# xeTaiz/vit-tf

Measured on AMD Instinct MI355X. Metric: slices/sec (ViT-S/8, 512^3 vol: feature volume + 16-query similarity), higher is better.
Workload: dtype fp16; 1 GPU; 512^3 CT-like synthetic volume (seed 0), ViT-S/8, fos 64: 1536 slices of 512x512 (N=4097) per step + 16-query similarity -> the metric's configuration (BASELINE configs[2]); engine_batch=512, weights=seeded synthetic vits8 (seed 0), parallelism=single GPU

## Files before the change

### vit-tf_amd/csrc/tail_fx.hip

```cpp
#include "vittf_common.h"

#include <type_traits>
#include <utility>

namespace {

constexpr int D = 384, HID = 4 * D, UNITS = HID / 32;
constexpr int SB = 24576, HB = SB / 2;
constexpr int PSTEPS = D / 32;
constexpr int LAG = 4;
constexpr int MSTEPS = 2 * UNITS + LAG;
constexpr int NSEQ = PSTEPS + MSTEPS;
constexpr int NSLOT = 4, AHEAD = NSLOT - 1;
constexpr int PIECES = SB / 1024 / 4;
constexpr int WAIT0 = (AHEAD - 2) * PIECES;
constexpr int NF = 4;
constexpr int PB_OFF = NSLOT * SB;
constexpr int PBH = 4608, PB = 2 * PBH;
constexpr int STG_ROW = 144;
constexpr int AF_SLOT = 1056, AF_H = 528;
constexpr int CONST_OFF = PB_OFF + 4 * PB;
constexpr int C_B1 = 0, C_B2 = HID, C_G1 = HID + D, C_E1 = HID + 2 * D,
              C_BP = HID + 3 * D, C_G2 = HID + 4 * D, C_E2 = HID + 5 * D,
              C_N = HID + 6 * D;
// ... 177 lines not shown
#define FX_ROLE_ENV                                                                                                       \
  const unsigned short* const abuf = uni_ptr(c.abuf);                                                                     \
  float* const x = uni_ptr(c.x);                                                                                          \
  unsigned short* const hout = uni_ptr(c.hout);                                                                           \
  unsigned* const tile_ctr = uni_ptr(c.tile_ctr);                                                                         \
  const int64_t rows = (int64_t)(((uint64_t)uni((unsigned)((uint64_t)c.rows >> 32)) << 32) | uni((unsigned)c.rows));     \
  const float ln_eps = __uint_as_float(uni(__float_as_uint(c.ln_eps)));                                                   \
  const int ntiles = (int)uni((unsigned)c.ntiles);                                                                        \
  int tile = (int)uni((unsigned)c.tile);                                                                                  \
  const unsigned lds0 = uni(c.lds0);                                                                                      \
  const int tid = threadIdx.x;                                                                                            \
  const int lane = tid & 63, wave = __builtin_amdgcn_readfirstlane(tid >> 6);                                             \
  const int rb = wave & 3;                                                                                                \
  const int h = lane >> 5, l31 = lane & 31;                                                                               \
  unsigned cl = lds0 + CONST_OFF + 16 * h;                                                                                \
  asm volatile("" : "+v"(cl));                                                                                            \
  auto cst4 = [&](int i) { return *(lds_f4_ptr)(cl + 4 * i); };             \
  const unsigned nxt = lds0 + NEXT_OFF;                                                                                   \
  Ring st;                                                                                                                \
  st.rsrc = lds_dma_rsrc(uni_ptr(c.wpk), (unsigned)(NSEQ * SB));                                                          \
  st.src0 = rb * (PIECES * 1024);                                                                                         \
  st.dma_dst = lds0;                                                                                                      \
  st.g = 0;                                                                                                               \
  st.slot = 0;                                                                                                            \
  const int aoff0 = tile_off(l31, h);                                                                                     \
  const unsigned pbuf = lds0 + PB_OFF + rb * PB;                           \
   \
  auto tile_rsrc = [&](const void* p, int64_t tile, int row_bytes) {                                                      \
    const int64_t first = tile * 128, left = rows - first;                                                                \
    const int nrows = tile < 0 || left <= 0 || !p ? 0 : left < 128 ? (int)left : 128;                                     \
    return __builtin_amdgcn_make_buffer_rsrc(const_cast<char*>(reinterpret_cast<const char*>(p)) + (nrows ? first : 0) * row_bytes, 0, \
                                             nrows * row_bytes, 0x00020000);                                              \
  };                                                                                                                      \
  (void)abuf; (void)x; (void)hout; (void)tile_ctr; (void)ln_eps; (void)ntiles; (void)l31; (void)aoff0; (void)nxt; (void)cst4; (void)tile_rsrc

template <int DT>
__device__ __attribute__((noinline)) void run_f(Ctx c) {
  FX_ROLE_ENV;
  asm volatile("s_setprio 3");
  unsigned pbl = pbuf + lane * 16;
  asm volatile("" : "+v"(pbl));
  u32x4_t fb[48];
  const int q8 = lane >> 3, c8 = lane & 7;
  __amdgpu_buffer_rsrc_t ra, rx;
  const int ao = (rb * 32 + q8) * (D * 2) + c8 * 16, xo = (rb * 32 + q8) * (D * 4) + c8 * 16;
  auto load_a = [&](int cg) {
#pragma unroll
    for (int i = 0; i < 4; ++i) fb[4 * cg + i] = __builtin_amdgcn_raw_buffer_load_b128(ra, ao + cg * 128, i * 8 * (D * 2), 0);
  };
  auto load_chunk = [&](int c) {
    const int r0 = c < 6 ? 24 + 4 * c : 4 * (c - 6);
#pragma unroll
    for (int i = 0; i < 4; ++i) fb[r0 + i] = __builtin_amdgcn_raw_buffer_load_b128(rx, xo + c * 128, i * 8 * (D * 4), 0);
  };
  const unsigned af_wr = pbuf + (c8 >> 1) * AF_SLOT + (c8 & 1) * AF_H + q8 * 16;
  auto put_a = [&](int cg) {
#pragma unroll
    for (int i = 0; i < 4; ++i) *(lds_wu4_ptr)(af_wr + af_off(4 * cg) + i * 128) = fb[4 * cg + i];
  };
  const unsigned ch_wr = pbuf + q8 * STG_ROW + c8 * 16;
  auto put_chunk = [&](int c) {
    const int r0 = c < 6 ? 24 + 4 * c : 4 * (c - 6);
#pragma unroll
    for (int i = 0; i < 4; ++i) *(lds_wu4_ptr)(ch_wr + (c & 1) * PBH + i * 8 * STG_ROW) = fb[r0 + i];
  };
  auto fetch_rows = [&](int t) {
    ra = tile_rsrc(abuf, t, D * 2);
    rx = tile_rsrc(x, t, D * 4);
#pragma unroll
    for (int cg = 0; cg < 6; ++cg) load_a(cg);
#pragma unroll
    for (int c = 0; c < 6; ++c) load_chunk(c);
    put_a(0);
  };
  fetch_rows(tile);
  asm volatile("s_waitcnt vmcnt(0)" ::: "memory");
  __syncthreads();
  while (true) {
    unsigned next_v = 0;
    if (tid == 256) next_v = atomicAdd(tile_ctr, 1u);
    unsigned base[4];
    s16x8_t hf[D / 16];
    s16x8_t wf[NF];
    f32x16_t bias_c;
    auto load_bias = [&](int at) {
#pragma unroll
      for (int q = 0; q < 4; ++q) {
        const f32x4_t bv = cst4(at + 8 * q);
        bias_c[4 * q + 0] = bv[0]; bias_c[4 * q + 1] = bv[1]; bias_c[4 * q + 2] = bv[2]; bias_c[4 * q + 3] = bv[3];
      }
    };
#pragma unroll
    for (int p = 0; p < PSTEPS; ++p) {
      sync_wait<true>();
      if (p % 2 == 0 && p / 2 + 1 < 6) put_a(p / 2 + 1);
      if (p == 0) load_chunk(6);
      if (p % 2 == 1 && p / 2 < 5) load_chunk(7 + p / 2);
      if (p == PSTEPS - 1) put_chunk(0);
      ring_advance(st);
    }
#pragma unroll
    for (int r = 0; r < 12; ++r) {
      sync_wait<true>();
      if (r + 1 < 12) put_chunk(r + 1);
    }
#pragma unroll
    for (int r = 0; r < 12; ++r) {
      sync_wait<true>();
// ... 19 lines not shown
      __builtin_amdgcn_sched_barrier(0);
    }
    ring_advance(st);
    f_step<DT, 1, false, false, false>(st, base, wf, hf, ga, bias_c, gb, pk1);
    for (int u = 1; u < UNITS - 1; u += 2) {
      load_bias(C_B1 + 32 * u);
      f_step<DT, 0, true, false, true>(st, base, wf, hf, gb, bias_c, ga, pk0);
      f_step<DT, 1, true, false, false>(st, base, wf, hf, gb, bias_c, ga, pk1);
      put_gf(0);
      load_bias(C_B1 + 32 * (u + 1));
      f_step<DT, 0, true, false, true>(st, base, wf, hf, ga, bias_c, gb, pk0);
      f_step<DT, 1, true, false, false>(st, base, wf, hf, ga, bias_c, gb, pk1);
      put_gf(1);
    }
    load_bias(C_B1 + 32 * (UNITS - 1));
    f_step<DT, 0, true, false, true>(st, base, wf, hf, gb, bias_c, ga, pk0);
    f_step<DT, 1, true, true, false>(st, base, wf, hf, gb, bias_c, ga, pk1);
    put_gf(0);
    sync_wait<true>();
    ring_advance(st);
#pragma unroll
    for (int r = 0; r < 16; r += 2) {
      const float v0 = gelu_poly(gb[r]), v1 = gelu_poly(gb[r + 1]);
      const unsigned w = pack2_h16<DT>(v0, v1);
      if (r < 8) pk0[r >> 1] = w; else pk1[(r - 8) >> 1] = w;
    }
    put_gf(1);
    sync_wait<true>(); ring_advance(st);
    sync_wait(); ring_advance(st);
    sync_wait(); ring_advance(st);
    if (tid == 256) *(lds_u32_ptr)nxt = next_v;
    asm volatile("s_waitcnt vmcnt(0) lgkmcnt(0)\n\ts_barrier" ::: "memory");
    const int next = __builtin_amdgcn_readfirstlane((int)*(lds_u32_ptr)nxt);
    if (next >= ntiles) break;
    tile = next;
    fetch_rows(tile);
  }
}

template <int DT>
__device__ __attribute__((noinline)) void run_x(Ctx c) {
  FX_ROLE_ENV;
  unsigned base[4];
  asm volatile("s_waitcnt vmcnt(0)" ::: "memory");
  __syncthreads();
  s16x8_t wf[NF];
  f32x16_t xacc[D / 32];
  while (true) {
    int ln = lane;
    asm volatile("" : "+v"(ln));
    {
#pragma unroll
      for (int ot = 0; ot < D / 32; ++ot)
#pragma unroll
        for (int q = 0; q < 4; ++q) {
          const f32x4_t bv = cst4(C_BP + 32 * ot + 8 * q);
          xacc[ot][4 * q + 0] = bv[0]; xacc[ot][4 * q + 1] = bv[1]; xacc[ot][4 * q + 2] = bv[2]; xacc[ot][4 * q + 3] = bv[3];
        }
#pragma unroll
      for (int i = 0; i < 4; ++i) base[i] = lds0 + st.slot * SB + (aoff0 ^ (32 * i));
      const unsigned af_rd = pbuf + (ln >> 5) * AF_H + (ln & 31) * 16;
      s16x8_t aa[2], ab[2];
      x_wait<-1, true>();
#pragma unroll
      for (int f = 0; f < NF; ++f) wf[f] = ld_frag(base, f);
      aa[0] = *(lds_frag_ptr)(af_rd + af_off(0));
      aa[1] = *(lds_frag_ptr)(af_rd + af_off(1));
      p_step<DT, -1, true, false>(st, base, wf, xacc, aa, ab, af_rd + af_off(2), af_rd + af_off(3));
      p_step<DT, -1, false, false>(st, base, wf, xacc, ab, aa, af_rd + af_off(4), af_rd + af_off(5));
// ... 64 lines not shown
          }
          *(lds_wu4_ptr)(hw_ + (ot & 1) * PBH + k2 * 1024) = pk;
        }
        sync_wait<true>();
      }
    }
    s16x8_t gf[2];
    x_idle_step<WAIT0>(st); x_idle_step<WAIT0>(st); x_idle_step<WAIT0>(st);
    x_wait<WAIT0>();
    {
      const int g_next = ring_next(st), slot_free = ring_free(st);
#pragma unroll
      for (int i = 0; i < PIECES; ++i) ring_piece(st, i, g_next, slot_free);
      ring_advance(st);
#pragma unroll
      for (int i = 0; i < 4; ++i) base[i] = lds0 + st.slot * SB + HB + (aoff0 ^ (32 * i));
#pragma unroll
      for (int f = 0; f < NF; ++f) wf[f] = ld_frag(base, f);
    }
    const unsigned gfa = pbuf + ln * 16;
    for (int u = 0; u < UNITS - 2; u += 2) {
      x_step<DT, 0, false>(st, base, wf, xacc, gf, gfa);
      x_step<DT, 1, false>(st, base, wf, xacc, gf, gfa);
      x_step<DT, 0, false>(st, base, wf, xacc, gf, gfa + PBH);
      x_step<DT, 1, false>(st, base, wf, xacc, gf, gfa + PBH);
    }
    x_step<DT, 0, false>(st, base, wf, xacc, gf, gfa);
    x_step<DT, 1, false>(st, base, wf, xacc, gf, gfa);
    x_step<DT, 0, false>(st, base, wf, xacc, gf, gfa + PBH);
    x_step<DT, 1, true>(st, base, wf, xacc, gf, gfa + PBH);
    asm volatile("s_waitcnt vmcnt(0) lgkmcnt(0)\n\ts_barrier" ::: "memory");
    const int next = __builtin_amdgcn_readfirstlane((int)*(lds_u32_ptr)nxt);
    {
      const auto rxo = tile_rsrc(x, tile, D * 4);
      const auto rho = tile_rsrc(hout, tile, D * 2);
      int le = lane;
      asm volatile("" : "+v"(le));
      const unsigned stg_wr_e = pbuf + (le & 31) * STG_ROW + 16 * (le >> 5);
      const unsigned stg_wh = pbuf + (le & 31) * STG_ROW + 8 * (le >> 5);
      const unsigned stg_rd_e = pbuf + (le >> 3) * STG_ROW + (le & 7) * 16;
      const int xo_e = (rb * 32 + (le >> 3)) * (D * 4) + (le & 7) * 16;
      const int ho = (rb * 32 + (le >> 3)) * (D * 2) + (le & 7) * 16;
      float s = 0.f;
      {
        f32x4_t bvq[2][4];
#pragma unroll
        for (int g = 0; g < 4; ++g) bvq[0][g] = cst4(C_B2 + 8 * g);
#pragma unroll
        for (int ot = 0; ot < D / 32; ++ot) {
#pragma unroll
          for (int g = 0; g < 4; ++g) {
            const f32x4_t bv = bvq[ot & 1][g];
            f32x4_t v;
            v[0] = xacc[ot][4 * g + 0] + bv[0]; v[1] = xacc[ot][4 * g + 1] + bv[1];
            v[2] = xacc[ot][4 * g + 2] + bv[2]; v[3] = xacc[ot][4 * g + 3] + bv[3];
#pragma unroll
            for (int e = 0; e < 4; ++e) xacc[ot][4 * g + e] = v[e];
            *(lds_w4_ptr)(stg_wr_e + 32 * g) = v;
            s += (v[0] + v[1]) + (v[2] + v[3]);
          }
          __builtin_amdgcn_sched_barrier(0);
          f32x4_t rbk[4];
#pragma unroll
          for (int i = 0; i < 4; ++i) rbk[i] = *(lds_f4_ptr)(stg_rd_e + i * 8 * STG_ROW);
          if (ot + 1 < D / 32) {
#pragma unroll
            for (int g = 0; g < 4; ++g) bvq[(ot + 1) & 1][g] = cst4(C_B2 + 32 * (ot + 1) + 8 * g);
          }
          __builtin_amdgcn_sched_barrier(0);
#pragma unroll
          for (int i = 0; i < 4; ++i)
            __builtin_amdgcn_raw_buffer_store_b128(__builtin_bit_cast(u32x4_t, rbk[i]), rxo, xo_e + ot * 128, i * 8 * (D * 4), 0);
          __builtin_amdgcn_sched_barrier(0);
        }
      }
      if (hout) {
        {
          const auto sw = __builtin_amdgcn_permlane32_swap(__float_as_uint(s), __float_as_uint(s), false, false);
          s = __uint_as_float(sw[0]) + __uint_as_float(sw[1]);
        }
        const float mean = s / (float)D;
        float q = 0.f;
#pragma unroll
        for (int ot = 0; ot < D / 32; ++ot) {
#pragma unroll
          for (int r = 0; r < 16; ++r) { const float dv = xacc[ot][r] - mean; q += dv * dv; }
          __builtin_amdgcn_sched_barrier(0);
        }
        {
          const auto sw = __builtin_amdgcn_permlane32_swap(__float_as_uint(q), __float_as_uint(q), false, false);
          q = __uint_as_float(sw[0]) + __uint_as_float(sw[1]);
        }
        const float rstd = 1.0f / sqrtf(q / (float)D + ln_eps);
        float mean_p = mean;
        asm volatile("" : "+v"(mean_p));
        f32x4_t gq1[2][4], bq1[2][4];
#pragma unroll
        for (int g = 0; g < 4; ++g) { gq1[0][g] = cst4(C_G1 + 8 * g); bq1[0][g] = cst4(C_E1 + 8 * g); }
#pragma unroll
        for (int ot = 0; ot < D / 32; ++ot) {
          const int op = ot >> 1, o2 = ot & 1;
#pragma unroll
          for (int g = 0; g < 4; ++g) {
            const f32x4_t gg = gq1[ot & 1][g], bb = bq1[ot & 1][g];
            u32x2_t pk;
            pk[0] = pack2_h16<DT>((xacc[ot][4 * g + 0] - mean_p) * rstd * gg[0] + bb[0], (xacc[ot][4 * g + 1] - mean_p) * rstd * gg[1] + bb[1]);
            pk[1] = pack2_h16<DT>((xacc[ot][4 * g + 2] - mean_p) * rstd * gg[2] + bb[2], (xacc[ot][4 * g + 3] - mean_p) * rstd * gg[3] + bb[3]);
            *(lds_w2_ptr)(stg_wh + 64 * o2 + 16 * g) = pk;
          }
          __builtin_amdgcn_sched_barrier(0);
          [[maybe_unused]] f32x4_t rbk[4];
          if (o2) {
#pragma unroll
            for (int i = 0; i < 4; ++i) rbk[i] = *(lds_f4_ptr)(stg_rd_e + i * 8 * STG_ROW);
          }
          if (ot + 1 < D / 32) {
#pragma unroll
            for (int g = 0; g < 4; ++g) { gq1[(ot + 1) & 1][g] = cst4(C_G1 + 32 * (ot + 1) + 8 * g); bq1[(ot + 1) & 1][g] = cst4(C_E1 + 32 * (ot + 1) + 8 * g); }
          }
          __builtin_amdgcn_sched_barrier(0);
          if (o2) {
#pragma unroll
            for (int i = 0; i < 4; ++i)
              __builtin_amdgcn_raw_buffer_store_b128(__builtin_bit_cast(u32x4_t, rbk[i]), rho, ho + op * 128, i * 8 * (D * 2), 0);
            __builtin_amdgcn_sched_barrier(0);
          }
        }
      }
    }
    if (next >= ntiles) break;
    tile = next;
  }
}

template <int DT>
__global__ __launch_bounds__(512, 1) void tail_fx_kernel(const unsigned short* __restrict__ abuf, const unsigned short* __restrict__ wpk,
                                                         const float* __restrict__ bp, const float* __restrict__ g2, const float* __restrict__ e2,
                                                         const float* __restrict__ b1, const float* __restrict__ b2,
                                                         float* __restrict__ x, int64_t rows, const float* __restrict__ ln_g,
                                                         const float* __restrict__ ln_b, float ln_eps,
                                                         unsigned short* __restrict__ hout, int ntiles,
                                                         unsigned* __restrict__ tile_ctr) {
  __shared__ __attribute__((aligned(16))) char smem[LDS_BYTES];
  const int tid = threadIdx.x;
  const int lane = tid & 63, wave = __builtin_amdgcn_readfirstlane(tid >> 6);
  float* const cst = reinterpret_cast<float*>(smem + CONST_OFF);
  for (int i = tid; i < C_N; i += 512) {
    float v;
    if (i < C_B2) v = b1[i];
    else if (i < C_G1) v = b2[i - C_B2];
    else if (i < C_E1) v = ln_g ? ln_g[i - C_G1] : 1.f;
    else if (i < C_BP) v = ln_b ? ln_b[i - C_E1] : 0.f;
    else if (i < C_G2) v = bp[i - C_BP];
    else if (i < C_E2) v = g2[i - C_G2];
    else v = e2[i - C_E2];
    cst[i] = v;
  }
  const unsigned lds0 = (unsigned)(size_t)LDS_PTR(smem);
  const unsigned nxt = lds0 + NEXT_OFF;
  if (tid == 0) *(lds_u32_ptr)nxt = atomicAdd(tile_ctr, 1u);
  __syncthreads();
  const int tile = __builtin_amdgcn_readfirstlane((int)*(lds_u32_ptr)nxt);
  if (tile >= ntiles) return;
  if (wave < 4) {
// ... 46 lines not shown
```

### include/vittf.h

```cpp
#ifndef VITTF_H
#define VITTF_H

#include <stddef.h>
#include <stdint.h>

#ifdef __cplusplus
extern "C" {
#endif

#define VITTF_ABI_VERSION 6

typedef enum vittf_status {
  VITTF_OK = 0,
  VITTF_ERR_INVALID_ARG = -1,
  VITTF_ERR_WORKSPACE = -2,
  VITTF_ERR_LAUNCH = -3,
  VITTF_ERR_NO_DEVICE = -4
} vittf_status;

typedef enum vittf_dtype { VITTF_BF16 = 0, VITTF_FP16 = 1 } vittf_dtype;

typedef enum vittf_axis { VITTF_AXIS_X = 0, VITTF_AXIS_Y = 1, VITTF_AXIS_Z = 2 } vittf_axis;

typedef enum vittf_sample_mode { VITTF_SAMPLE_NEAREST = 0, VITTF_SAMPLE_TRILINEAR = 1 } vittf_sample_mode;
// ... 114 lines not shown
                          float* tokens_out, void* stream);

int vittf_layernorm(const float* x, const float* g, const float* b, void* y, int64_t rows, int32_t d,
                    float eps, int32_t dtype, void* stream);

int vittf_token_features(const float* x, const float* norm_g, const float* norm_b, uint16_t* t_out, int32_t batch,
                         int32_t tokens, int32_t prefix, int32_t d, float eps, void* stream);

typedef enum vittf_epilogue {
  VITTF_EPI_BIAS = 0,
  VITTF_EPI_BIAS_GELU = 1,
  VITTF_EPI_BIAS_RESIDUAL = 2,
  VITTF_EPI_KFEAT = 3,
  VITTF_EPI_BIAS_QKV = 4
} vittf_epilogue;

int vittf_gemm(const void* a, const void* w, const float* bias, void* out, int64_t rows, int32_t n, int32_t k,
               int32_t epilogue, int32_t tokens, int32_t dtype, void* stream);

int vittf_gemm_kfeat_parts(const void* a, const void* w, const float* bias, int64_t rows, int32_t d, int32_t k,
                           int32_t tokens, int32_t part_mask, void* q_out, void* k_out, void* v_out, int32_t dtype,
                           void* stream);

int vittf_gemm_kfeat_parts_reg(const void* a, const void* w, const float* bias, int64_t rows, int32_t d, int32_t k,
                               int32_t tokens, int32_t n_reg, int32_t part_mask, void* q_out, void* k_out, void* v_out,
                               int32_t dtype, void* stream);

int vittf_gemm_residual_ln(const void* a, const void* w, const float* bias, float* x, int64_t rows, int32_t n, int32_t k,
                           int32_t dtype, const float* ln_g, const float* ln_b, float ln_eps, void* h, void* stream);

size_t vittf_gemm_as_workspace_bytes(void);
int vittf_gemm_as(const void* a, const void* w_packed, const float* bias, void* out, int64_t rows, int32_t n, int32_t k,
                  int32_t epilogue, int32_t dtype, void* tile_counter, void* stream);

size_t vittf_block_tail_workspace_bytes(void);
int vittf_block_tail(const void* attn_out, const void* w_packed, const float* proj_b, const float* ln2_g, const float* ln2_b,
                     const float* b1, const float* b2, float* x, int64_t rows, int32_t d, int32_t dtype, const float* ln_g,
                     const float* ln_b, float ln_eps, void* h_out, void* tile_counter, void* stream);

int vittf_rope_qk(void* qkv, int64_t rows, int32_t tokens, int32_t prefix, int32_t heads, const vittf_rope_table* table,
                  int32_t dtype, void* stream);

int vittf_attention(const void* qkv, void* out, int32_t batch, int32_t tokens, int32_t heads, int32_t dtype,
                    int32_t q_prescaled, void* stream);

int64_t vittf_attention_rescale_count(int32_t reset);

size_t vittf_attention_fp8_workspace_bytes(int32_t batch, int32_t tokens, int32_t heads);
int vittf_attention_fp8(const void* qkv, void* out, int32_t batch, int32_t tokens, int32_t heads, int32_t dtype, void* ws,
                        size_t ws_bytes, void* stream);

int vittf_gemm_qkv_fp8(const void* a, const void* w, const float* bias, void* qkv_out, int64_t rows, int32_t n, int32_t k,
                       int32_t tokens, int32_t heads, int32_t dtype, void* ws, size_t ws_bytes, void* stream);
int vittf_attention_fp8_rows(const void* qkv, void* out, int32_t batch, int32_t tokens, int32_t heads, int32_t dtype, void* ws,
                             size_t ws_bytes, void* stream);


int vittf_pool_slices(const uint16_t* k_slices, int32_t k_slice0, int32_t k_nslices, int32_t total_slices,
                      int32_t n_out, int32_t win0, int32_t nwin, int32_t f0, int32_t f1, int32_t d,
                      uint16_t* dst, int64_t dst_stride_d, int64_t dst_stride_win, int64_t dst_stride_row,
                      int64_t dst_stride_col, void* stream);

int vittf_pool_slices3d(const uint16_t* k_slices, int32_t k_slice0, int32_t k_nslices, int32_t total_slices,
                        int32_t n_out, int32_t win0, int32_t nwin, int32_t f0, int32_t f1, int32_t d,
                        uint16_t* dst, int64_t dst_stride_d, int64_t dst_stride_win, int64_t dst_stride_row,
                        int64_t dst_stride_col, int32_t o0, int32_t o1, int32_t slice_dim, void* stream);
// ... 94 lines not shown
```

### vit-tf_amd/_lib.py

```python
import ctypes as C
import os

_HERE = os.path.dirname(os.path.abspath(__file__))
LIB_PATH = os.path.join(_HERE, 'libvittf.so')

BF16, FP16 = 0, 1
DTYPES = {'bf16': BF16, 'bfloat16': BF16, 'fp16': FP16, 'float16': FP16, 'half': FP16}
SAMPLE_MODES = {'nearest': 0, 'bilinear': 1, 'trilinear': 1}
EPI_BIAS, EPI_BIAS_GELU, EPI_BIAS_RESIDUAL, EPI_KFEAT, EPI_BIAS_QKV = 0, 1, 2, 3, 4


class VitConfig(C.Structure):
    _fields_ = [('embed_dim', C.c_int32), ('depth', C.c_int32), ('heads', C.c_int32), ('patch', C.c_int32),
                ('dtype', C.c_int32), ('ln_eps', C.c_float), ('attention_fp8', C.c_int32), ('flags', C.c_int32)]


CFG_SEPARATE_LN, CFG_UNSCALED_Q, CFG_FP8_HEAD_SCALES = 1, 2, 4


class VitWeights(C.Structure):
    _fields_ = [(n, C.c_void_p) for n in (
        'pe_w_t', 'pe_b', 'qkv_w', 'qkv_b', 'proj_w', 'proj_b', 'fc1_w', 'fc1_b', 'fc2_w', 'fc2_b', 'tail_packed', 'qkv_packed',
        'ln1_g', 'ln1_b', 'ln2_g', 'ln2_b')]

# ... 28 lines not shown
SIGNATURES = {
    'vittf_abi_version': (C.c_int, []),
    'vittf_status_string': (C.c_char_p, [C.c_int]),
    'vittf_device_count': (C.c_int, []),
    'vittf_minmax_workspace_bytes': (_sz, []),
    'vittf_volume_minmax': (C.c_int, [_vp, _i64, _vp, _vp, _sz, _vp]),
    'vittf_vit_workspace_bytes': (_sz, [_P(VitConfig), _i32, _i32]),
    'vittf_vit_k_features': (C.c_int, [_P(VitConfig), _P(VitWeights), _P(PosEmbed), _P(SliceView), _i32, _i32, _i32,
                                       _vp, _vp, _sz, _vp]),
    'vittf_vit_qkv_features': (C.c_int, [_P(VitConfig), _P(VitWeights), _P(PosEmbed), _P(SliceView), _i32, _i32, _i32,
                                         _vp, _vp, _vp, _vp, _sz, _vp]),
    'vittf_vit_qkv_features_reg': (C.c_int, [_P(VitConfig), _P(VitWeights), _P(PosEmbed), _P(SliceView), _i32, _i32, _i32,
                                             _vp, _i32, _vp, _vp, _vp, _vp, _sz, _vp]),
    'vittf_vit_qkv_features_rope': (C.c_int, [_P(VitConfig), _P(VitWeights), _P(PosEmbed), _P(SliceView), _i32, _i32, _i32,
                                              _vp, _i32, _P(RopeTable), _vp, _vp, _vp, _vp, _sz, _vp]),
    'vittf_vit_features': (C.c_int, [_P(VitConfig), _P(VitWeights), _P(PosEmbed), _P(SliceView), _i32, _i32, _i32, _vp, _i32,
                                     _P(RopeTable), _vp, _vp, _vp, _vp, _vp, _vp, _vp, _sz, _vp]),
    'vittf_profiler_enable': (C.c_int, [_i32]),
    'vittf_profiler_collect': (C.c_int, [_P(C.c_double), _P(_i64)]),
    'vittf_profiler_kernel_name': (C.c_char_p, [_i32]),
    'vittf_patch_embed': (C.c_int, [_P(VitConfig), _P(VitWeights), _P(PosEmbed), _P(SliceView), _i32, _i32, _vp, _vp]),
    'vittf_patch_embed_reg': (C.c_int, [_P(VitConfig), _P(VitWeights), _P(PosEmbed), _P(SliceView), _i32, _i32, _vp, _i32, _vp,
                                        _vp]),
    'vittf_token_features': (C.c_int, [_vp, _vp, _vp, _vp, _i32, _i32, _i32, _i32, C.c_float, _vp]),
    'vittf_layernorm': (C.c_int, [_vp, _vp, _vp, _vp, _i64, _i32, C.c_float, _i32, _vp]),
    'vittf_gemm': (C.c_int, [_vp, _vp, _vp, _vp, _i64, _i32, _i32, _i32, _i32, _i32, _vp]),
    'vittf_gemm_kfeat_parts': (C.c_int, [_vp, _vp, _vp, _i64, _i32, _i32, _i32, _i32, _vp, _vp, _vp, _i32, _vp]),
    'vittf_gemm_kfeat_parts_reg': (C.c_int, [_vp, _vp, _vp, _i64, _i32, _i32, _i32, _i32, _i32, _vp, _vp, _vp, _i32, _vp]),
    'vittf_gemm_residual_ln': (C.c_int, [_vp, _vp, _vp, _vp, _i64, _i32, _i32, _i32, _vp, _vp, C.c_float, _vp, _vp]),
    'vittf_block_tail_workspace_bytes': (_sz, []),
    'vittf_block_tail': (C.c_int, [_vp, _vp, _vp, _vp, _vp, _vp, _vp, _vp, _i64, _i32, _i32, _vp, _vp, C.c_float, _vp, _vp, _vp]),
    'vittf_gemm_as_workspace_bytes': (_sz, []),
    'vittf_gemm_as': (C.c_int, [_vp, _vp, _vp, _vp, _i64, _i32, _i32, _i32, _i32, _vp, _vp]),
    'vittf_rope_qk': (C.c_int, [_vp, _i64, _i32, _i32, _i32, _P(RopeTable), _i32, _vp]),
    'vittf_attention': (C.c_int, [_vp, _vp, _i32, _i32, _i32, _i32, _i32, _vp]),
    'vittf_attention_rescale_count': (_i64, [_i32]),
    'vittf_attention_fp8_workspace_bytes': (_sz, [_i32, _i32, _i32]),
    'vittf_attention_fp8': (C.c_int, [_vp, _vp, _i32, _i32, _i32, _i32, _vp, _sz, _vp]),
    'vittf_gemm_qkv_fp8': (C.c_int, [_vp, _vp, _vp, _vp, _i64, _i32, _i32, _i32, _i32, _i32, _vp, _sz, _vp]),
    'vittf_attention_fp8_rows': (C.c_int, [_vp, _vp, _i32, _i32, _i32, _i32, _vp, _sz, _vp]),
    'vittf_pool_slices': (C.c_int, [_vp, _i32, _i32, _i32, _i32, _i32, _i32, _i32, _i32, _i32, _vp, _i64, _i64, _i64,
                                    _i64, _vp]),
    'vittf_pool_slices3d': (C.c_int, [_vp, _i32, _i32, _i32, _i32, _i32, _i32, _i32, _i32, _i32, _vp, _i64, _i64, _i64,
                                      _i64, _i32, _i32, _i32, _vp]),
    'vittf_assemble_sum': (C.c_int, [_vp, _vp, _vp, _i32, _P(_i32), _i32, _i32, _i32, _i32, _vp, _vp]),
    'vittf_sample_features': (C.c_int, [_vp, _i32, _i32, _i32, _i32, _i32, _vp, _i32, _i32, _vp, _vp, _vp]),
    'vittf_voxel_norm': (C.c_int, [_vp, _i32, _i64, _vp, _vp]),
    'vittf_similarity_workspace_bytes': (_sz, [_i32, _i64, _i32]),
    'vittf_similarity': (C.c_int, [_vp, _i32, _i32, _i32, _i32, _vp, _P(_i32), _i32, _i32, _vp, _i32, _i32, _i32, _vp, _vp,
                                   _sz, _vp]),
    'vittf_similarity_query_workspace_bytes': (_sz, [_i32, _i64, _i32, _i32]),
    'vittf_similarity_query': (C.c_int, [_vp, _i32, _i32, _i32, _i32, _P(C.c_float), _P(_i32), _i32, _i32, _vp, _i32, _i32, _i32,
                                         _vp, _vp, _sz, _vp]),
    'vittf_similarity_maps_f32': (C.c_int, [_vp, _i32, _i32, _i32, _i32, _i32, _vp, _P(_i32), _i32, _i32, C.c_float, _vp, _vp,
                                            _vp, _sz, _vp]),
    'vittf_feature_gram_workspace_bytes': (_sz, [_i32, _i64]),
    'vittf_feature_gram': (C.c_int, [_vp, _i32, _i64, _vp, _vp, _vp, _sz, _vp]),
    'vittf_feature_project': (C.c_int, [_vp, _i32, _i64, _vp, _vp, _i32, _vp, _vp]),
    'vittf_kmeans_assign': (C.c_int, [_vp, _i32, _i64, _vp, _vp, _i32, _vp, _vp, _vp]),
    'vittf_kmeans_sums_workspace_bytes': (_sz, [_i32, _i64, _i32]),
    'vittf_kmeans_sums': (C.c_int, [_vp, _i32, _i64, _vp, _i32, _vp, _vp, _vp, _sz, _vp]),
    'vittf_topk_voxels': (C.c_int, [_vp, _i32, _i64, _i32, _vp, _vp]),
    'vittf_mean_pairwise_distance': (C.c_int, [_vp, _i32, _i32, _i32, _vp, _vp]),
    'vittf_erode_mask': (C.c_int, [_vp, _i32, _i32, _i32, _i32, _i32, _vp, _vp]),
    'vittf_surface_shell_workspace_bytes': (_sz, [_i32, _i32, _i32]),
    'vittf_surface_shell': (C.c_int, [_vp, _i32, _i32, _i32, _i32, _i32, _vp, _vp, _sz, _vp]),
# ... 84 lines not shown
```

### vit-tf_amd/csrc/gemm_as.hip

```cpp
#include "vittf_common.h"

#include <stdlib.h>
#include <type_traits>

namespace {

constexpr int K = 384;
constexpr int SB = 24576;
constexpr int NSLOT = 4, AHEAD = NSLOT - 1;
constexpr int PIECES = SB / 1024 / 4;
constexpr int NF = 4;
constexpr int STG_ROW = 144, STG = 32 * STG_ROW;
constexpr int STG_OFF = NSLOT * SB;
constexpr int BIAS_OFF = STG_OFF + 12 * STG;
constexpr int MAXN = 1536;
constexpr int NEXT_OFF = BIAS_OFF + MAXN * 4;
constexpr int LDS_BYTES = NEXT_OFF + 16;
static_assert(LDS_BYTES <= 160 * 1024, "LDS");

typedef __attribute__((ext_vector_type(4))) unsigned u32x4_t;
typedef __attribute__((ext_vector_type(2))) unsigned u32x2_t;
typedef __attribute__((address_space(3))) const s16x8_t* lds_frag_ptr;
typedef __attribute__((address_space(3))) const f32x4_t* lds_f4_ptr;
typedef __attribute__((address_space(3))) u32x2_t* lds_w2_ptr;
typedef __attribute__((address_space(3))) volatile unsigned* lds_u32_ptr;

__device__ __forceinline__ void lds_dma16_keep(i32x4_t rsrc, unsigned lds_addr, int voff, int soff) {
  asm volatile("s_mov_b32 m0, %0\n\ts_nop 0\n\tbuffer_load_dwordx4 %1, %2, %3 offen lds"
               :: "s"(lds_addr), "v"(voff), "s"(rsrc), "s"(soff) : "memory");
}

template <int DT>
__global__ __launch_bounds__(512, 1) void gemm_as_kernel(const unsigned short* __restrict__ abuf, const unsigned short* __restrict__ wpk,
                                                         const float* __restrict__ bias, unsigned short* __restrict__ out, int64_t rows,
                                                         int n, int qcols, int ntiles, unsigned* __restrict__ tile_ctr) {
  __shared__ __attribute__((aligned(16))) char smem[LDS_BYTES];
  const int tid = threadIdx.x;
  const int lane = tid & 63, wave = __builtin_amdgcn_readfirstlane(tid >> 6);
  const int h = lane >> 5, l31 = lane & 31, q8 = lane >> 3, c8 = lane & 7;
  const unsigned lds0 = (unsigned)(size_t)LDS_PTR(smem);
  float* const cst = reinterpret_cast<float*>(smem + BIAS_OFF);
  for (int i = tid; i < n; i += 512) cst[i] = bias[i];
  const unsigned nxt = lds0 + NEXT_OFF;
  if (tid == 0) *(lds_u32_ptr)nxt = atomicAdd(tile_ctr, 1u);
  __syncthreads();
  int tile = __builtin_amdgcn_readfirstlane((int)*(lds_u32_ptr)nxt);
  if (tile >= ntiles) return;
  const int units = n >> 5;
  const i32x4_t rsrc = lds_dma_rsrc(wpk, (unsigned)(units * SB));
  const bool storer = wave >= 4;
  const int src0 = (wave & 3) * (PIECES * 1024);
  if (!storer) {
#pragma unroll
    for (int u = 0; u < AHEAD; ++u)
#pragma unroll
      for (int i = 0; i < PIECES; ++i)
        lds_dma16(rsrc, lds0 + u * SB + src0 + i * 1024, lane * 16, u * SB + src0 + i * 1024);
  }
  int g = 0, slot = 0;
  const int aoff0 = tile_off(l31, h);
  unsigned base[4];
#pragma unroll
  for (int i = 0; i < 4; ++i) base[i] = lds0 + (aoff0 ^ (32 * i));
  const unsigned stg = lds0 + STG_OFF + (storer ? 8 + (wave - 4) : 2 * wave) * STG;
  const unsigned stg_w = stg + l31 * STG_ROW + 8 * h;
  const unsigned stg_r = stg + q8 * STG_ROW + c8 * 16;
  const unsigned stg_rp = lds0 + STG_OFF + 2 * (wave & 3) * STG + q8 * STG_ROW + c8 * 16;
  unsigned cl = lds0 + BIAS_OFF + 16 * h;
  asm volatile("" : "+v"(cl));
  constexpr float QS = 0.125f * 1.44269504088896340736f;
  asm volatile("s_waitcnt vmcnt(0)" ::: "memory");
  __syncthreads();
  s16x8_t wf[NF];
#pragma unroll
  for (int f = 0; f < NF; ++f) wf[f] = *(lds_frag_ptr)(base[f & 3] + (f >> 2) * 4096);
  const int row_bytes_out = n * 2;

  while (true) {
    unsigned next_v = 0;
    if (tid == 256) next_v = atomicAdd(tile_ctr, 1u);
    const int64_t first = (int64_t)tile * 256, left = rows - first;
    const int nrows = left < 256 ? (int)left : 256;
    const auto ra = __builtin_amdgcn_make_buffer_rsrc(const_cast<unsigned short*>(abuf) + first * K, 0, nrows * (K * 2), 0x00020000);
    const auto ro = __builtin_amdgcn_make_buffer_rsrc(out + first * n, 0, nrows * row_bytes_out, 0x00020000);
    s16x8_t hq[K / 16];
#pragma unroll
    for (int s = 0; s < K / 16; ++s)
      hq[s] = __builtin_bit_cast(s16x8_t, __builtin_amdgcn_raw_buffer_load_b128(ra, (wave * 32 + l31) * (K * 2) + 16 * h, 32 * s, 0));
    const int oo = (wave * 32 + q8) * row_bytes_out + c8 * 16;
    f32x16_t qa = {}, qb = {};
    f32x4_t ba[4], bb[4];
    auto load_bias = [&](int u, f32x4_t (&b)[4]) {
#pragma unroll
      for (int gq = 0; gq < 4; ++gq) b[gq] = *(lds_f4_ptr)(cl + 4 * (32 * u + 8 * gq));
    };
    auto stage = [&](const f32x16_t& q, const f32x4_t (&bq)[4], int u, int gq) {
      const f32x4_t b = bq[gq];
      const float qsc = 32 * u < qcols ? QS : 1.f;
      u32x2_t pk;
      pk[0] = pack2_h16<DT>((q[4 * gq + 0] + b[0]) * qsc, (q[4 * gq + 1] + b[1]) * qsc);
      pk[1] = pack2_h16<DT>((q[4 * gq + 2] + b[2]) * qsc, (q[4 * gq + 3] + b[3]) * qsc);
      *(lds_w2_ptr)(stg_w + (storer ? 0 : ((u >> 1) & 1) * STG) + 64 * (u & 1) + 16 * gq) = pk;
    };
    auto store_pair = [&](int m, bool partner) {
      if (!storer) return;
      const unsigned rd = partner ? stg_rp + (m & 1) * STG : stg_r;
      f32x4_t rbk[4];
#pragma unroll
      for (int i = 0; i < 4; ++i) rbk[i] = *(lds_f4_ptr)(rd + i * 8 * STG_ROW);
#pragma unroll
      for (int i = 0; i < 4; ++i)
        __builtin_amdgcn_raw_buffer_store_b128(__builtin_bit_cast(u32x4_t, rbk[i]), ro, oo + (partner ? -128 * row_bytes_out : 0) + m * 128,
                                               i * 8 * row_bytes_out, 0);
    };
    auto unit = [&](auto WAITc, f32x16_t& acc, f32x4_t (&bcur)[4], const f32x16_t& prevq, const f32x4_t (&bprev)[4], int u, bool stage_prev) {
      constexpr int WAITN = decltype(WAITc)::value;
      load_bias(u, bcur);
      if (storer) asm volatile("s_waitcnt lgkmcnt(0)\n\ts_barrier" ::: "memory");
      else asm volatile("s_waitcnt vmcnt(%0) lgkmcnt(0)\n\ts_barrier" ::"i"(WAITN) : "memory");
      if (u >= 3 && (u & 1)) store_pair((u - 3) >> 1, true);
      const int g_next = g + AHEAD < units ? g + AHEAD : g + AHEAD - units;
      const int slot_free = slot == 0 ? NSLOT - 1 : slot - 1;
#pragma unroll
      for (int j = 0; j < 24; ++j) {
        acc = mfma32<DT>(wf[j % NF], hq[j], j == 0 ? f32x16_t{} : acc);
        if (j == 24 - NF) {
          const int d_ = slot == NSLOT - 1 ? -(NSLOT - 1) * SB : SB;
#pragma unroll
          for (int i = 0; i < 4; ++i) { base[i] += d_; asm volatile("" : "+v"(base[i])); }
        }
        wf[j % NF] = *(lds_frag_ptr)(base[((j + NF) % 24) & 3] + (((j + NF) % 24) >> 2) * 4096);
        if (!storer && j % 4 == 3) lds_dma16_keep(rsrc, lds0 + slot_free * SB + src0 + (j >> 2) * 1024, lane * 16, g_next * SB + src0 + (j >> 2) * 1024);
        if (stage_prev && j % 6 == 2) stage(prevq, bprev, u - 1, j / 6);
        __builtin_amdgcn_sched_barrier(0);
      }
      g = g + 1 == units ? 0 : g + 1;
      slot = slot + 1 == NSLOT ? 0 : slot + 1;
    };
    using W6 = std::integral_constant<int, PIECES>;
    using WT = std::integral_constant<int, PIECES + K / 16>;
    unit(WT{}, qa, ba, qb, bb, 0, false);
    unit(W6{}, qb, bb, qa, ba, 1, true);
    for (int u = 2; u < units; u += 2) {
      unit(W6{}, qa, ba, qb, bb, u, true);
      store_pair((u - 2) >> 1, false);
      unit(W6{}, qb, bb, qa, ba, u + 1, true);
    }
#pragma unroll
    for (int gq = 0; gq < 4; ++gq) stage(qb, bb, units - 1, gq);
    store_pair((units - 2) >> 1, false);
    if (tid == 256) *(lds_u32_ptr)nxt = next_v;
    asm volatile("s_waitcnt lgkmcnt(0)\n\ts_barrier" ::: "memory");
    store_pair((units - 2) >> 1, true);
    const int next = __builtin_amdgcn_readfirstlane((int)*(lds_u32_ptr)nxt);
    if (next >= ntiles) break;
    tile = next;
  }
  asm volatile("s_waitcnt vmcnt(0)" ::: "memory");
}

}

extern "C" size_t vittf_gemm_as_workspace_bytes(void) { return sizeof(unsigned); }

extern "C" int vittf_gemm_as(const void* a, const void* w_packed, const float* bias, void* out, int64_t rows, int32_t n, int32_t k,
                             int32_t epilogue, int32_t dtype, void* tile_counter, void* stream) {
  if (!a || !w_packed || !bias || !out || rows <= 0) return VITTF_ERR_INVALID_ARG;
  if (k != K || n <= 0 || n % 64 != 0 || n > MAXN) return VITTF_ERR_INVALID_ARG;
  if (epilogue != VITTF_EPI_BIAS && epilogue != VITTF_EPI_BIAS_QKV) return VITTF_ERR_INVALID_ARG;
  if (epilogue == VITTF_EPI_BIAS_QKV && n % 96 != 0) return VITTF_ERR_INVALID_ARG;
  if ((((uintptr_t)a | (uintptr_t)w_packed | (uintptr_t)out | (uintptr_t)bias) & 15) != 0) return VITTF_ERR_INVALID_ARG;
  if (!tile_counter || ((uintptr_t)tile_counter & 3) != 0) return VITTF_ERR_INVALID_ARG;
  const int64_t tiles = (rows + 255) / 256;
  if (tiles > 0x7fffff) return VITTF_ERR_INVALID_ARG;
  const int cus = vittf_current_cus();
  if (cus <= 0) return VITTF_ERR_NO_DEVICE;
  const unsigned grid = (unsigned)(tiles < cus ? tiles : cus);
  hipStream_t st = (hipStream_t)stream;
  unsigned* ctr = (unsigned*)tile_counter;
  if (hipMemsetAsync(ctr, 0, sizeof(unsigned), st) != hipSuccess) return VITTF_ERR_LAUNCH;
  const int qcols = epilogue == VITTF_EPI_BIAS_QKV ? n / 3 : 0;
#define AS_LAUNCH(DTV)                                                                                               \
  hipLaunchKernelGGL((gemm_as_kernel<DTV>), dim3(grid), dim3(512), 0, st, (const unsigned short*)a,                  \
                     (const unsigned short*)w_packed, bias, (unsigned short*)out, rows, (int)n, qcols, (int)tiles, ctr)
  if (dtype == VITTF_BF16) AS_LAUNCH(VITTF_BF16);
  else if (dtype == VITTF_FP16) AS_LAUNCH(VITTF_FP16);
  else return VITTF_ERR_INVALID_ARG;
#undef AS_LAUNCH
  vittf_note_kernel(VITTF_KERNEL_GEMM_QKV, "gemm_as_kernel");
  return vittf_check_launch();
}
```

Baseline: 2306 slices/s.

## Move tail epilogue global stores from x-role waves to f-role waves

The x-role waves now only write the residual and LayerNorm results into double-buffered LDS staging and signal via sync_wait, instead of reading them back and issuing the global stores themselves. The f-role waves, after prefetching the next tile's rows, read the staged chunks and issue the buffer stores for x and hout. This aims to shorten the x-role epilogue critical path and overlap output writes with the next tile's input loads. In exchange it adds extra named-barrier handshakes per chunk and makes the f-role waves do more work, and it relies on the two roles staying in lockstep with matching sync counts.

```diff
diff --git a/vit-tf_amd/csrc/tail_fx.hip b/vit-tf_amd/csrc/tail_fx.hip
--- a/vit-tf_amd/csrc/tail_fx.hip
+++ b/vit-tf_amd/csrc/tail_fx.hip
@@ -233,7 +233,7 @@
     return __builtin_amdgcn_make_buffer_rsrc(const_cast<char*>(reinterpret_cast<const char*>(p)) + (nrows ? first : 0) * row_bytes, 0, \
                                              nrows * row_bytes, 0x00020000);                                              \
   };                                                                                                                      \
-  (void)abuf; (void)x; (void)hout; (void)tile_ctr; (void)ln_eps; (void)ntiles; (void)l31; (void)aoff0; (void)nxt; (void)cst4; (void)tile_rsrc
+  (void)abuf; (void)x; (void)hout; (void)tile_ctr; (void)ln_eps; (void)ntiles; (void)l31; (void)aoff0; (void)nxt; (void)cst4; (void)tile_rsrc; (void)tile
 
 template <int DT>
 __device__ __attribute__((noinline)) void run_f(Ctx c) {
@@ -265,16 +265,24 @@
 #pragma unroll
     for (int i = 0; i < 4; ++i) *(lds_wu4_ptr)(ch_wr + (c & 1) * PBH + i * 8 * STG_ROW) = fb[r0 + i];
   };
-  auto fetch_rows = [&](int t) {
+  auto load_rows = [&](int t) {
     ra = tile_rsrc(abuf, t, D * 2);
     rx = tile_rsrc(x, t, D * 4);
 #pragma unroll
     for (int cg = 0; cg < 6; ++cg) load_a(cg);
 #pragma unroll
     for (int c = 0; c < 6; ++c) load_chunk(c);
-    put_a(0);
   };
-  fetch_rows(tile);
+  auto store_round = [&](int half, __amdgpu_buffer_rsrc_t rs, int off, int row_bytes) {
+    sync_wait<true>();
+    u32x4_t rbk[4];
+#pragma unroll
+    for (int i = 0; i < 4; ++i) rbk[i] = *(lds_wu4_ptr)(ch_wr + half * PBH + i * 8 * STG_ROW);
+#pragma unroll
+    for (int i = 0; i < 4; ++i) __builtin_amdgcn_raw_buffer_store_b128(rbk[i], rs, off, i * 8 * row_bytes, 0);
+  };
+  load_rows(tile);
+  put_a(0);
   asm volatile("s_waitcnt vmcnt(0)" ::: "memory");
   __syncthreads();
   while (true) {
@@ -360,9 +368,18 @@
     if (tid == 256) *(lds_u32_ptr)nxt = next_v;
     asm volatile("s_waitcnt vmcnt(0) lgkmcnt(0)\n\ts_barrier" ::: "memory");
     const int next = __builtin_amdgcn_readfirstlane((int)*(lds_u32_ptr)nxt);
+    const auto rxo = tile_rsrc(x, tile, D * 4);
+    const auto rho = tile_rsrc(hout, tile, D * 2);
+    load_rows(next);
+#pragma unroll
+    for (int ot = 0; ot < D / 32; ++ot) store_round(ot & 1, rxo, xo + ot * 128, D * 4);
+    if (hout) {
+#pragma unroll
+      for (int op = 0; op < D / 64; ++op) store_round(op & 1, rho, ao + op * 128, D * 2);
+    }
     if (next >= ntiles) break;
     tile = next;
-    fetch_rows(tile);
+    put_a(0);
   }
 }
 
@@ -493,15 +510,10 @@
     asm volatile("s_waitcnt vmcnt(0) lgkmcnt(0)\n\ts_barrier" ::: "memory");
     const int next = __builtin_amdgcn_readfirstlane((int)*(lds_u32_ptr)nxt);
     {
-      const auto rxo = tile_rsrc(x, tile, D * 4);
-      const auto rho = tile_rsrc(hout, tile, D * 2);
       int le = lane;
       asm volatile("" : "+v"(le));
       const unsigned stg_wr_e = pbuf + (le & 31) * STG_ROW + 16 * (le >> 5);
       const unsigned stg_wh = pbuf + (le & 31) * STG_ROW + 8 * (le >> 5);
-      const unsigned stg_rd_e = pbuf + (le >> 3) * STG_ROW + (le & 7) * 16;
-      const int xo_e = (rb * 32 + (le >> 3)) * (D * 4) + (le & 7) * 16;
-      const int ho = (rb * 32 + (le >> 3)) * (D * 2) + (le & 7) * 16;
       float s = 0.f;
       {
         f32x4_t bvq[2][4];
@@ -517,22 +529,15 @@
             v[2] = xacc[ot][4 * g + 2] + bv[2]; v[3] = xacc[ot][4 * g + 3] + bv[3];
 #pragma unroll
             for (int e = 0; e < 4; ++e) xacc[ot][4 * g + e] = v[e];
-            *(lds_w4_ptr)(stg_wr_e + 32 * g) = v;
+            *(lds_w4_ptr)(stg_wr_e + (ot & 1) * PBH + 32 * g) = v;
             s += (v[0] + v[1]) + (v[2] + v[3]);
           }
           __builtin_amdgcn_sched_barrier(0);
-          f32x4_t rbk[4];
-#pragma unroll
-          for (int i = 0; i < 4; ++i) rbk[i] = *(lds_f4_ptr)(stg_rd_e + i * 8 * STG_ROW);
           if (ot + 1 < D / 32) {
 #pragma unroll
             for (int g = 0; g < 4; ++g) bvq[(ot + 1) & 1][g] = cst4(C_B2 + 32 * (ot + 1) + 8 * g);
           }
-          __builtin_amdgcn_sched_barrier(0);
-#pragma unroll
-          for (int i = 0; i < 4; ++i)
-            __builtin_amdgcn_raw_buffer_store_b128(__builtin_bit_cast(u32x4_t, rbk[i]), rxo, xo_e + ot * 128, i * 8 * (D * 4), 0);
-          __builtin_amdgcn_sched_barrier(0);
+          sync_wait<true>();
         }
       }
       if (hout) {
@@ -567,30 +572,18 @@
             u32x2_t pk;
             pk[0] = pack2_h16<DT>((xacc[ot][4 * g + 0] - mean_p) * rstd * gg[0] + bb[0], (xacc[ot][4 * g + 1] - mean_p) * rstd * gg[1] + bb[1]);
             pk[1] = pack2_h16<DT>((xacc[ot][4 * g + 2] - mean_p) * rstd * gg[2] + bb[2], (xacc[ot][4 * g + 3] - mean_p) * rstd * gg[3] + bb[3]);
-            *(lds_w2_ptr)(stg_wh + 64 * o2 + 16 * g) = pk;
+            *(lds_w2_ptr)(stg_wh + (op & 1) * PBH + 64 * o2 + 16 * g) = pk;
           }
           __builtin_amdgcn_sched_barrier(0);
-          [[maybe_unused]] f32x4_t rbk[4];
-          if (o2) {
-#pragma unroll
-            for (int i = 0; i < 4; ++i) rbk[i] = *(lds_f4_ptr)(stg_rd_e + i * 8 * STG_ROW);
-          }
           if (ot + 1 < D / 32) {
 #pragma unroll
             for (int g = 0; g < 4; ++g) { gq1[(ot + 1) & 1][g] = cst4(C_G1 + 32 * (ot + 1) + 8 * g); bq1[(ot + 1) & 1][g] = cst4(C_E1 + 32 * (ot + 1) + 8 * g); }
           }
-          __builtin_amdgcn_sched_barrier(0);
-          if (o2) {
-#pragma unroll
-            for (int i = 0; i < 4; ++i)
-              __builtin_amdgcn_raw_buffer_store_b128(__builtin_bit_cast(u32x4_t, rbk[i]), rho, ho + op * 128, i * 8 * (D * 2), 0);
-            __builtin_amdgcn_sched_barrier(0);
-          }
+          if (o2) sync_wait<true>();
         }
       }
     }
     if (next >= ntiles) break;
-    tile = next;
   }
 }
 
```

Result: no change. 2305 slices/s (-0.0%).

## Split GEMM tiles into column work items to balance persistent-kernel tail

Applied to the files above, without the earlier changes.

Replaces whole-tile scheduling in the persistent QKV GEMM with work items that can cover a column range of a tile. The first tiles are staggered into head/remainder pieces and the leftover partial wave of tiles is sliced across columns, so CUs finish together instead of idling in the last wave. A/activation loads are restaged through LDS with coalesced loads, and next-item prefetch is moved earlier into the unit pipeline. This adds decode logic, extra work items and redundant A-tile loads per split tile, and alters the weight ring indexing, which risks correctness if the slot/image mapping is wrong.

```diff
diff --git a/include/vittf.h b/include/vittf.h
--- a/include/vittf.h
+++ b/include/vittf.h
@@ -170,6 +170,7 @@
 size_t vittf_gemm_as_workspace_bytes(void);
 int vittf_gemm_as(const void* a, const void* w_packed, const float* bias, void* out, int64_t rows, int32_t n, int32_t k,
                   int32_t epilogue, int32_t dtype, void* tile_counter, void* stream);
+int vittf_gemm_as_plan(int64_t rows, int32_t n, int32_t* grid, int32_t* heads, int32_t* full_tiles, int32_t* slices);
 
 size_t vittf_block_tail_workspace_bytes(void);
 int vittf_block_tail(const void* attn_out, const void* w_packed, const float* proj_b, const float* ln2_g, const float* ln2_b,
diff --git a/vit-tf_amd/_lib.py b/vit-tf_amd/_lib.py
--- a/vit-tf_amd/_lib.py
+++ b/vit-tf_amd/_lib.py
@@ -84,6 +84,7 @@
     'vittf_block_tail': (C.c_int, [_vp, _vp, _vp, _vp, _vp, _vp, _vp, _vp, _i64, _i32, _i32, _vp, _vp, C.c_float, _vp, _vp, _vp]),
     'vittf_gemm_as_workspace_bytes': (_sz, []),
     'vittf_gemm_as': (C.c_int, [_vp, _vp, _vp, _vp, _i64, _i32, _i32, _i32, _i32, _vp, _vp]),
+    'vittf_gemm_as_plan': (C.c_int, [_i64, _i32, _P(_i32), _P(_i32), _P(_i32), _P(_i32)]),
     'vittf_rope_qk': (C.c_int, [_vp, _i64, _i32, _i32, _i32, _P(RopeTable), _i32, _vp]),
     'vittf_attention': (C.c_int, [_vp, _vp, _i32, _i32, _i32, _i32, _i32, _vp]),
     'vittf_attention_rescale_count': (_i64, [_i32]),
diff --git a/vit-tf_amd/csrc/gemm_as.hip b/vit-tf_amd/csrc/gemm_as.hip
--- a/vit-tf_amd/csrc/gemm_as.hip
+++ b/vit-tf_amd/csrc/gemm_as.hip
@@ -23,6 +23,7 @@
 typedef __attribute__((address_space(3))) const s16x8_t* lds_frag_ptr;
 typedef __attribute__((address_space(3))) const f32x4_t* lds_f4_ptr;
 typedef __attribute__((address_space(3))) u32x2_t* lds_w2_ptr;
+typedef __attribute__((address_space(3))) u32x4_t* lds_w4_ptr;
 typedef __attribute__((address_space(3))) volatile unsigned* lds_u32_ptr;
 
 __device__ __forceinline__ void lds_dma16_keep(i32x4_t rsrc, unsigned lds_addr, int voff, int soff) {
@@ -33,7 +34,7 @@
 template <int DT>
 __global__ __launch_bounds__(512, 1) void gemm_as_kernel(const unsigned short* __restrict__ abuf, const unsigned short* __restrict__ wpk,
                                                          const float* __restrict__ bias, unsigned short* __restrict__ out, int64_t rows,
-                                                         int n, int qcols, int ntiles, unsigned* __restrict__ tile_ctr) {
+                                                         int n, int qcols, int nitems, int nhead, int nfull, int slices, unsigned* __restrict__ tile_ctr) {
   __shared__ __attribute__((aligned(16))) char smem[LDS_BYTES];
   const int tid = threadIdx.x;
   const int lane = tid & 63, wave = __builtin_amdgcn_readfirstlane(tid >> 6);
@@ -44,20 +45,43 @@
   const unsigned nxt = lds0 + NEXT_OFF;
   if (tid == 0) *(lds_u32_ptr)nxt = atomicAdd(tile_ctr, 1u);
   __syncthreads();
-  int tile = __builtin_amdgcn_readfirstlane((int)*(lds_u32_ptr)nxt);
-  if (tile >= ntiles) return;
+  const int item = __builtin_amdgcn_readfirstlane((int)*(lds_u32_ptr)nxt);
+  if (item >= nitems) return;
   const int units = n >> 5;
+  auto decode = [&](int it, int& t, int& first_unit, int& item_units) {
+    const int pairs = units >> 1;
+    t = it, first_unit = 0, item_units = units;
+    if (it < nhead) {
+      item_units = 2 * (2 + it * (pairs - 3) / nhead);
+    } else if (it >= nfull && it < nfull + nhead) {
+      t = it - nfull;
+      first_unit = 2 * (2 + t * (pairs - 3) / nhead), item_units = units - first_unit;
+    } else if (it >= nfull + nhead && it < nitems) {
+      const int kk = it - nfull - nhead, lt = kk / slices, sl = kk - lt * slices;
+      const int p0 = sl * pairs / slices, p1 = (sl + 1) * pairs / slices;
+      t = nfull + lt, first_unit = 2 * p0, item_units = 2 * (p1 - p0);
+    }
+  };
+  int tile, u0, nu;
+  decode(item, tile, u0, nu);
+  auto image_of = [&](int t, int u0n) {
+    const int x = u0n + t - nu;
+    return t < nu ? u0 + t : x < units ? x : x - units;
+  };
   const i32x4_t rsrc = lds_dma_rsrc(wpk, (unsigned)(units * SB));
   const bool storer = wave >= 4;
   const int src0 = (wave & 3) * (PIECES * 1024);
   if (!storer) {
 #pragma unroll
-    for (int u = 0; u < AHEAD; ++u)
+    for (int u = 0; u < AHEAD; ++u) {
+      const int img = image_of(u, 0);
 #pragma unroll
       for (int i = 0; i < PIECES; ++i)
-        lds_dma16(rsrc, lds0 + u * SB + src0 + i * 1024, lane * 16, u * SB + src0 + i * 1024);
+        lds_dma16(rsrc, lds0 + u * SB + src0 + i * 1024, lane * 16, img * SB + src0 + i * 1024);
+    }
   }
-  int g = 0, slot = 0;
+  int slot = 0;
+  int hb = 0;
   const int aoff0 = tile_off(l31, h);
   unsigned base[4];
 #pragma unroll
@@ -84,19 +108,34 @@
     const auto ra = __builtin_amdgcn_make_buffer_rsrc(const_cast<unsigned short*>(abuf) + first * K, 0, nrows * (K * 2), 0x00020000);
     const auto ro = __builtin_amdgcn_make_buffer_rsrc(out + first * n, 0, nrows * row_bytes_out, 0x00020000);
     s16x8_t hq[K / 16];
-#pragma unroll
-    for (int s = 0; s < K / 16; ++s)
-      hq[s] = __builtin_bit_cast(s16x8_t, __builtin_amdgcn_raw_buffer_load_b128(ra, (wave * 32 + l31) * (K * 2) + 16 * h, 32 * s, 0));
-    const int oo = (wave * 32 + q8) * row_bytes_out + c8 * 16;
+    {
+      u32x4_t fb[K / 16];
+      const int ao = (wave * 32 + q8) * (K * 2) + c8 * 16;
+#pragma unroll
+      for (int cg = 0; cg < 6; ++cg)
+#pragma unroll
+        for (int i = 0; i < 4; ++i) fb[4 * cg + i] = __builtin_amdgcn_raw_buffer_load_b128(ra, ao + cg * 128, i * 8 * (K * 2), 0);
+      const unsigned hbuf = stg + (storer ? 0 : hb * STG);
+      const unsigned hw = hbuf + q8 * STG_ROW + c8 * 16, hr = hbuf + l31 * STG_ROW + 16 * h;
+#pragma unroll
+      for (int cg = 0; cg < 6; ++cg) {
+#pragma unroll
+        for (int i = 0; i < 4; ++i) *(lds_w4_ptr)(hw + i * 8 * STG_ROW) = fb[4 * cg + i];
+#pragma unroll
+        for (int i = 0; i < 4; ++i) hq[4 * cg + i] = *(lds_frag_ptr)(hr + 32 * i);
+      }
+    }
+    const int oo = (wave * 32 + q8) * row_bytes_out + u0 * 64 + c8 * 16;
+    int next = nitems, tile_n = 0, u0n = 0, nun = 0;
     f32x16_t qa = {}, qb = {};
     f32x4_t ba[4], bb[4];
     auto load_bias = [&](int u, f32x4_t (&b)[4]) {
 #pragma unroll
-      for (int gq = 0; gq < 4; ++gq) b[gq] = *(lds_f4_ptr)(cl + 4 * (32 * u + 8 * gq));
+      for (int gq = 0; gq < 4; ++gq) b[gq] = *(lds_f4_ptr)(cl + 4 * (32 * (u0 + u) + 8 * gq));
     };
     auto stage = [&](const f32x16_t& q, const f32x4_t (&bq)[4], int u, int gq) {
       const f32x4_t b = bq[gq];
-      const float qsc = 32 * u < qcols ? QS : 1.f;
+      const float qsc = 32 * (u0 + u) < qcols ? QS : 1.f;
       u32x2_t pk;
       pk[0] = pack2_h16<DT>((q[4 * gq + 0] + b[0]) * qsc, (q[4 * gq + 1] + b[1]) * qsc);
       pk[1] = pack2_h16<DT>((q[4 * gq + 2] + b[2]) * qsc, (q[4 * gq + 3] + b[3]) * qsc);
@@ -113,13 +152,18 @@
         __builtin_amdgcn_raw_buffer_store_b128(__builtin_bit_cast(u32x4_t, rbk[i]), ro, oo + (partner ? -128 * row_bytes_out : 0) + m * 128,
                                                i * 8 * row_bytes_out, 0);
     };
-    auto unit = [&](auto WAITc, f32x16_t& acc, f32x4_t (&bcur)[4], const f32x16_t& prevq, const f32x4_t (&bprev)[4], int u, bool stage_prev) {
-      constexpr int WAITN = decltype(WAITc)::value;
+    auto unit = [&](auto POSc, auto WAITc, f32x16_t& acc, f32x4_t (&bcur)[4], const f32x16_t& prevq, const f32x4_t (&bprev)[4], int u, bool stage_prev) {
+      constexpr int WAITN = decltype(WAITc)::value, POS = decltype(POSc)::value;
       load_bias(u, bcur);
       if (storer) asm volatile("s_waitcnt lgkmcnt(0)\n\ts_barrier" ::: "memory");
       else asm volatile("s_waitcnt vmcnt(%0) lgkmcnt(0)\n\ts_barrier" ::"i"(WAITN) : "memory");
+      if (POS == 0 && tid == 256) *(lds_u32_ptr)nxt = next_v;
+      if (POS == 1) {
+        next = __builtin_amdgcn_readfirstlane((int)*(lds_u32_ptr)nxt);
+        decode(next, tile_n, u0n, nun);
+      }
       if (u >= 3 && (u & 1)) store_pair((u - 3) >> 1, true);
-      const int g_next = g + AHEAD < units ? g + AHEAD : g + AHEAD - units;
+      const int g_next = image_of(u + AHEAD, u0n);
       const int slot_free = slot == 0 ? NSLOT - 1 : slot - 1;
 #pragma unroll
       for (int j = 0; j < 24; ++j) {
@@ -134,27 +178,27 @@
         if (stage_prev && j % 6 == 2) stage(prevq, bprev, u - 1, j / 6);
         __builtin_amdgcn_sched_barrier(0);
       }
-      g = g + 1 == units ? 0 : g + 1;
       slot = slot + 1 == NSLOT ? 0 : slot + 1;
     };
     using W6 = std::integral_constant<int, PIECES>;
-    using WT = std::integral_constant<int, PIECES + K / 16>;
-    unit(WT{}, qa, ba, qb, bb, 0, false);
-    unit(W6{}, qb, bb, qa, ba, 1, true);
-    for (int u = 2; u < units; u += 2) {
-      unit(W6{}, qa, ba, qb, bb, u, true);
+    using P0 = std::integral_constant<int, 0>;
+    using P1 = std::integral_constant<int, 1>;
+    using P2 = std::integral_constant<int, 2>;
+    unit(P0{}, W6{}, qa, ba, qb, bb, 0, false);
+    unit(P1{}, W6{}, qb, bb, qa, ba, 1, true);
+    for (int u = 2; u < nu; u += 2) {
+      unit(P2{}, W6{}, qa, ba, qb, bb, u, true);
       store_pair((u - 2) >> 1, false);
-      unit(W6{}, qb, bb, qa, ba, u + 1, true);
-    }
-#pragma unroll
-    for (int gq = 0; gq < 4; ++gq) stage(qb, bb, units - 1, gq);
-    store_pair((units - 2) >> 1, false);
-    if (tid == 256) *(lds_u32_ptr)nxt = next_v;
+      unit(P2{}, W6{}, qb, bb, qa, ba, u + 1, true);
+    }
+#pragma unroll
+    for (int gq = 0; gq < 4; ++gq) stage(qb, bb, nu - 1, gq);
+    store_pair((nu - 2) >> 1, false);
     asm volatile("s_waitcnt lgkmcnt(0)\n\ts_barrier" ::: "memory");
-    store_pair((units - 2) >> 1, true);
-    const int next = __builtin_amdgcn_readfirstlane((int)*(lds_u32_ptr)nxt);
-    if (next >= ntiles) break;
-    tile = next;
+    store_pair((nu - 2) >> 1, true);
+    if (next >= nitems) break;
+    hb = 1 ^ (((nu - 2) >> 1) & 1);
+    tile = tile_n, u0 = u0n, nu = nun;
   }
   asm volatile("s_waitcnt vmcnt(0)" ::: "memory");
 }
@@ -162,6 +206,21 @@
 }
 
 extern "C" size_t vittf_gemm_as_workspace_bytes(void) { return sizeof(unsigned); }
+
+extern "C" int vittf_gemm_as_plan(int64_t rows, int32_t n, int32_t* grid, int32_t* heads, int32_t* full_tiles, int32_t* slices) {
+  if (rows <= 0 || n <= 0 || n % 64 != 0 || n > MAXN || !grid || !heads || !full_tiles || !slices) return VITTF_ERR_INVALID_ARG;
+  const int64_t tiles = (rows + 255) / 256;
+  if (tiles > 0x7fffff) return VITTF_ERR_INVALID_ARG;
+  const int cus = vittf_current_cus();
+  if (cus <= 0) return VITTF_ERR_NO_DEVICE;
+  const int g = (int)(tiles < cus ? tiles : cus), r = (int)(tiles % g);
+  const int s = r ? (g / r < n / 128 ? g / r : n / 128) : 1;
+  *grid = g;
+  *slices = s >= 2 ? s : 1;
+  *full_tiles = (int)(s >= 2 ? tiles - r : tiles);
+  *heads = tiles >= 2 * (int64_t)g && n >= 256 ? g : 0;
+  return VITTF_OK;
+}
 
 extern "C" int vittf_gemm_as(const void* a, const void* w_packed, const float* bias, void* out, int64_t rows, int32_t n, int32_t k,
                              int32_t epilogue, int32_t dtype, void* tile_counter, void* stream) {
@@ -172,17 +231,17 @@
   if ((((uintptr_t)a | (uintptr_t)w_packed | (uintptr_t)out | (uintptr_t)bias) & 15) != 0) return VITTF_ERR_INVALID_ARG;
   if (!tile_counter || ((uintptr_t)tile_counter & 3) != 0) return VITTF_ERR_INVALID_ARG;
   const int64_t tiles = (rows + 255) / 256;
-  if (tiles > 0x7fffff) return VITTF_ERR_INVALID_ARG;
-  const int cus = vittf_current_cus();
-  if (cus <= 0) return VITTF_ERR_NO_DEVICE;
-  const unsigned grid = (unsigned)(tiles < cus ? tiles : cus);
+  int grid, nhead, nfull, slices;
+  const int prc = vittf_gemm_as_plan(rows, n, &grid, &nhead, &nfull, &slices);
+  if (prc != VITTF_OK) return prc;
+  const int nitems = nfull + nhead + (int)(tiles - nfull) * slices;
   hipStream_t st = (hipStream_t)stream;
   unsigned* ctr = (unsigned*)tile_counter;
   if (hipMemsetAsync(ctr, 0, sizeof(unsigned), st) != hipSuccess) return VITTF_ERR_LAUNCH;
   const int qcols = epilogue == VITTF_EPI_BIAS_QKV ? n / 3 : 0;
 #define AS_LAUNCH(DTV)                                                                                               \
   hipLaunchKernelGGL((gemm_as_kernel<DTV>), dim3(grid), dim3(512), 0, st, (const unsigned short*)a,                  \
-                     (const unsigned short*)w_packed, bias, (unsigned short*)out, rows, (int)n, qcols, (int)tiles, ctr)
+                     (const unsigned short*)w_packed, bias, (unsigned short*)out, rows, (int)n, qcols, nitems, nhead, nfull, slices, ctr)
   if (dtype == VITTF_BF16) AS_LAUNCH(VITTF_BF16);
   else if (dtype == VITTF_FP16) AS_LAUNCH(VITTF_FP16);
   else return VITTF_ERR_INVALID_ARG;
```

Measured after the change: 2285 slices/s before, 2281 slices/s after. About the same (-0.2%).
